# facebookresearch/r3m

Measured on AMD Instinct MI355X. Metric: encoder frames/sec (fwd+bwd) ResNet-50 224^2 bs=256/GPU, higher is better.
Workload: dtype f32

## Files before the change

### include/r3m_hip.h

```cpp
#ifndef R3M_HIP_H
#define R3M_HIP_H
#include <stddef.h>
#ifdef __cplusplus
extern "C" {
#endif

typedef void* r3m_stream_t;
typedef struct r3m_resnet* r3m_resnet_t;

int r3m_abi_version(void);
const char* r3m_last_error(void);

int r3m_debug_occupancy(int* out4);
int r3m_debug_occupy(int blocks, int lds_bytes, double milliseconds, r3m_stream_t stream);
int r3m_debug_set_dynamic_tiles(int on);
void r3m_debug_next_launch_tile_queues(unsigned* counters, int sets);
int r3m_debug_set_pw16(int mode);
int r3m_debug_set_conv3x3_bf16(int mode);
int r3m_debug_set_fused_inference(int on);
int r3m_debug_conv_route(int N, int H, int W, int Ci, int Co, int k, int stride, int pad, int dgrad, int flags, int mask_bits, int dtype,
                         int* routes, int cap);
int r3m_debug_conv_fuses_affine(int N, int H, int W, int Ci, int Co, int k, int stride, int pad, int flags, int dtype);
int r3m_debug_wgrad_route(int N, int H, int W, int Ci, int Co, int k, int stride, int pad, int dtype, int* out, int cap);
int r3m_debug_bn_geometry(long long rows, int C, int dtype, int* out, int cap);
void r3m_profile_enable(int on);
unsigned r3m_profile_classes(unsigned mask);
int r3m_profile_collect(double* ms, long long* launches, double* flops);
int r3m_profile_collect_bytes(double* bytes);
int r3m_profile_dump_to(const char* host_path);

r3m_resnet_t r3m_resnet_create(int size , int frames);
void r3m_resnet_destroy(r3m_resnet_t h);
int r3m_resnet_out_dim(r3m_resnet_t h);
long long r3m_resnet_num_params(r3m_resnet_t h);
long long r3m_resnet_num_buffers(r3m_resnet_t h);
long long r3m_resnet_arena_bytes(r3m_resnet_t h);
// ... 192 lines not shown
```

### r3m_amd/_lib.py

```python
import ctypes as C
import os

_HERE = os.path.dirname(os.path.abspath(__file__))
LIB_PATH = os.environ.get("R3M_HIP_LIB") or os.path.join(_HERE, "lib", "libr3m_hip.so")

_lib = None

c_f = C.c_void_p
c_i = C.c_int
c_ll = C.c_longlong
c_sz = C.c_size_t
c_fl = C.c_float
c_d = C.c_double

SIGNATURES = {
    "r3m_abi_version": (c_i, []),
    "r3m_last_error": (C.c_char_p, []),
    "r3m_debug_occupancy": (c_i, [C.POINTER(c_i)]),
    "r3m_debug_occupy": (c_i, [c_i, c_i, C.c_double, C.c_void_p]),
    "r3m_debug_set_dynamic_tiles": (c_i, [c_i]),
    "r3m_debug_next_launch_tile_queues": (None, [c_f, c_i]),
    "r3m_debug_set_pw16": (c_i, [c_i]),
    "r3m_debug_set_conv3x3_bf16": (c_i, [c_i]),
    "r3m_debug_set_fused_inference": (c_i, [c_i]),
    "r3m_debug_conv_route": (c_i, [c_i] * 12 + [C.POINTER(c_i), c_i]),
    "r3m_debug_wgrad_route": (c_i, [c_i] * 9 + [C.POINTER(c_i), c_i]),
    "r3m_debug_conv_fuses_affine": (c_i, [c_i] * 10),
    "r3m_debug_bn_geometry": (c_i, [c_ll, c_i, c_i, C.POINTER(c_i), c_i]),
    "r3m_profile_enable": (None, [c_i]),
    "r3m_profile_classes": (C.c_uint, [C.c_uint]),
    "r3m_profile_collect": (c_i, [C.POINTER(c_d), C.POINTER(c_ll), C.POINTER(c_d)]),
    "r3m_profile_collect_bytes": (c_i, [C.POINTER(c_d)]),
    "r3m_profile_dump_to": (c_i, [C.c_char_p]),
    "r3m_resnet_create": (C.c_void_p, [c_i, c_i]),
    "r3m_resnet_destroy": (None, [C.c_void_p]),
    "r3m_resnet_out_dim": (c_i, [C.c_void_p]),
    "r3m_resnet_num_params": (c_ll, [C.c_void_p]),
    "r3m_resnet_num_buffers": (c_ll, [C.c_void_p]),
    "r3m_resnet_arena_bytes": (c_ll, [C.c_void_p]),
    "r3m_resnet_num_tensors": (c_i, [C.c_void_p]),
# ... 189 lines not shown
```

### r3m_amd/csrc/capi.hip

```cpp
#include "engine.h"
#include "augment_dev.h"
#include "../../include/r3m_hip.h"
#include <cstdarg>
#include <cstdio>
#include <cstdlib>
#include <cstring>
#include <atomic>
#include <deque>
#include <mutex>
#include <string>
#include <vector>

namespace r3m {

static thread_local char g_err[512] = "";

void set_last_error(const char* fmt, ...) {
  va_list ap;
  va_start(ap, fmt);
  vsnprintf(g_err, sizeof g_err, fmt, ap);
  va_end(ap);
}

static int trace_mode() {
// ... 90 lines not shown
int r3m_debug_occupy(int blocks, int lds_bytes, double milliseconds, r3m_stream_t stream) {
  R3M_REQUIRE(blocks > 0 && lds_bytes >= 256 && lds_bytes <= 160 * 1024 && milliseconds >= 0.0, "debug_occupy: bad arguments");
  static r3m::DynLdsOptIn oi;
  if (int e = r3m::ensure_dyn_lds(oi, reinterpret_cast<const void*>(occupy_kernel), lds_bytes, "debug_occupy")) return e;
  hipLaunchKernelGGL(occupy_kernel, dim3(blocks), dim3(256), lds_bytes, static_cast<hipStream_t>(stream), (long long)(milliseconds * 1e5));
  return r3m::check_launch("debug_occupy");
}
int r3m_debug_set_dynamic_tiles(int on) { return r3m::gg_set_dynamic_tiles(on); }
void r3m_debug_next_launch_tile_queues(unsigned* counters, int sets) { r3m::gg_set_tile_counters(counters, counters && sets > 0 ? sets : 0); }
int r3m_debug_set_pw16(int mode) { return r3m::pw16_set_mode(mode); }
int r3m_debug_set_conv3x3_bf16(int mode) { return r3m::row16_set_mode(mode); }
int r3m_debug_set_fused_inference(int on) { return r3m::engine_set_fused_inference(on); }
int r3m_debug_conv_fuses_affine(int N, int H, int W, int Ci, int Co, int k, int stride, int pad, int flags, int dtype) {
  return r3m::conv_forward_affine_fusable({N, H, W, Ci, Co, k, stride, pad}, flags, dtype) ? 1 : 0;
}
int r3m_debug_conv_route(int N, int H, int W, int Ci, int Co, int k, int stride, int pad, int dgrad, int flags, int mask_bits, int dtype,
                         int* routes, int cap) {
  R3M_REQUIRE(routes && cap >= 1, "debug_conv_route: routes buffer");
  const unsigned* some_bits = reinterpret_cast<const unsigned*>(static_cast<uintptr_t>(64));
  const r3m::ConvGeom g{N, H, W, Ci, Co, k, stride, pad};
  r3m::gg_route_record_begin(routes, cap);
  int rc;
  if (!dgrad && (flags & EPI_AFFINE)) {
    const float* coef = reinterpret_cast<const float*>(some_bits);
    rc = r3m::conv_forward_launch_affine(nullptr, nullptr, nullptr, coef, coef, g, flags, dtype, nullptr);
  } else if (!dgrad) {
    rc = r3m::conv_forward_launch(nullptr, nullptr, nullptr, nullptr, nullptr, g, flags, dtype, nullptr);
  } else {
    r3m::BnRedArgs br{nullptr, mask_bits ? some_bits : nullptr, nullptr, nullptr, nullptr, nullptr, 0};
    const bool bn = (flags & 64) != 0;
    rc = r3m::conv_dgrad_launch(nullptr, nullptr, nullptr, nullptr, nullptr, (flags & 4) ? some_bits : nullptr, g, flags & ~64, dtype, nullptr,
                                bn ? &br : nullptr);
  }
  const int n = r3m::gg_route_record_end();
  return rc ? -1 : n;
}
int r3m_debug_wgrad_route(int N, int H, int W, int Ci, int Co, int k, int stride, int pad, int dtype, int* out, int cap) {
  if (!out || cap < 9) { r3m::set_last_error("debug_wgrad_route: the output buffer needs 9 ints"); return -1; }
  const r3m::WgradPlan r = r3m::conv_wgrad_plan({N, H, W, Ci, Co, k, stride, pad}, dtype);
  const int v[9] = {r.route, r.tile, r.bk, r.fast, r.split, r.rows_per_split, r.tilesN, r.gx, r.lds_bytes};
  for (int i = 0; i < 9; ++i) out[i] = v[i];
  return 9;
}
void r3m_profile_enable(int on) {
  std::lock_guard<std::mutex> lk(g_prof_mu);
  g_prof_on.store(on != 0, std::memory_order_relaxed);
  if (!on) g_prof_used = 0;
}
unsigned r3m_profile_classes(unsigned mask) { return g_prof_classes.exchange(mask, std::memory_order_relaxed); }
static FILE* g_prof_dump = nullptr;
// ... 554 lines not shown
```

### r3m_amd/csrc/common.h

```cpp
#pragma once
#include <hip/hip_runtime.h>
#include <stdint.h>
#include <stddef.h>

#ifdef R3M_PROBES
#include <cstdlib>
#define R3M_ENV_INT(name, dflt) ([]() -> int { static const int v_ = []() { const char* e_ = getenv(name); return e_ ? atoi(e_) : (dflt); }(); return v_; }())
#define R3M_PROBE(p) ((p).debug)
#else
#define R3M_ENV_INT(name, dflt) (dflt)
#define R3M_PROBE(p) 0
#endif

namespace r3m {

typedef float f32x4 __attribute__((ext_vector_type(4)));
typedef float f32x16 __attribute__((ext_vector_type(16)));

void set_last_error(const char* fmt, ...);
int  check_launch(const char* what);

#define R3M_REQUIRE(cond, ...)                  \
  do {                                          \
    if (!(cond)) {                              \
// ... 82 lines not shown
int launch_gather_gemm(const GatherGemmParams& p, hipStream_t s);
double gather_gemm_alg_bytes(const GatherGemmParams& p, int elem_bytes);
bool gather_gemm_fuses_affine(const GatherGemmParams& p);
int gather_gemm_grid_m(int M, int Nc);
void gg_set_tile_counters(unsigned* ctr8, int sets = 1);
int gg_set_dynamic_tiles(int on);
void gg_route_record_begin(int* out, int cap);
int gg_route_record_end();
struct WtEntry { long long w_off, wt_off; int Co, T, Ci, pad_; };
int launch_transpose_w_all(const float* params, void* wt, const WtEntry* tab, const int* tile0, int n, int tiles, int dt, hipStream_t s);
int launch_transpose_w(const float* W, float* Wt, int Co, int T, int Ci, hipStream_t s);

bool pw_gemm_eligible(const GatherGemmParams& p);
int pw_gemm_form(const GatherGemmParams& p);
int launch_pw_gemm(const GatherGemmParams& p, hipStream_t s);

enum : int {
  WG_TAPS_SIMPLE = 40,
  WG_TAPS_GATHER = 41,
  WG_ROWS        = 42,
  WG_WINDOW      = 43,
  WG16_TAPS      = 50,
  WG16_ROWS      = 51,
  WG16_ALL_TAPS  = 52,
};
struct WgradPlan {
  int route, tile, bk;
  int fast;
  int split, rows_per_split;
  int tilesN, gx;
// ... 151 lines not shown
```

### r3m_amd/csrc/conv.hip

```cpp
#include "common.h"
#include "conv_dev.h"
#include <utility>

namespace r3m {

__device__ __attribute__((aligned(128))) float g_zero_line[2048 + 64];


template <int EPI>
__global__ __launch_bounds__(256) void gather_gemm_glds_kernel(const GatherGemmParams p) {
  constexpr int BM = 128, BN = 128, WM = 2, WN = 2, TM = 2, TN = 2;
  constexpr int STAGE = (BM + BN) * 32;
  __shared__ __attribute__((aligned(128))) float smem[2 * STAGE];

  const int tid = threadIdx.x;
  const int lane = tid & 63;
  const int wave = tid >> 6;
  const int wm = wave / WN, wn = wave % WN;
  const int gridN = (p.Nc + BN - 1) / BN;
  const int lid = xcd_remap(blockIdx.x, gridDim.x);
  const int mt = lid / gridN, nt = lid % gridN;
  const int m0 = mt * BM, n0 = nt * BN;

  const int srow = lane >> 3;
// ... 749 lines not shown

  gg_epilogue<BM, BN, WM, WN, EPI, LDSB / 4>(p, acc, reinterpret_cast<float*>(wsm), m0, n0, mt);
}

static bool conv3x3_win_eligible(const GatherGemmParams& p, int maxW) {
  if (p.ntaps != 9 || p.is != 1 || p.os != 1 || p.simple_rows || p.Hg != p.Hi || p.Wg != p.Wi || p.Ho != p.Hi || p.Wo != p.Wi) return false;
  if (p.Wi > maxW || p.Wi < 1 || (p.Ci & 31)) return false;
  unsigned seen = 0;
  for (int t = 0; t < 9; ++t) {
    if (p.dy[t] < -1 || p.dy[t] > 1 || p.dx[t] < -1 || p.dx[t] > 1) return false;
    seen |= 1u << ((p.dy[t] + 1) * 3 + (p.dx[t] + 1));
  }
  return seen == 0x1ffu && (long long)p.Nc * p.T * p.Ci * 4 < 0x7FFFF000LL;
}

static inline bool gg_wide(int Nc) { return (Nc % 128) == 0; }

int gather_gemm_grid_m(int M, int Nc) { return gg_wide(Nc) ? ceil_div(M, 128) : ceil_div(M, 256); }

static int gg_use_glds() {
  const int v = R3M_ENV_INT("R3M_GG_GLDS", 2);
  return v;
}

#define GG_EPI_SWITCH(LAUNCH)                                                       \
  switch (p.flags) {                                                                \
    case 0: LAUNCH(0); break;                                                       \
    case EPI_STATS: LAUNCH(EPI_STATS); break;                                       \
    case EPI_ACCUM: LAUNCH(EPI_ACCUM); break;                                       \
    case EPI_MASKED_ADD: LAUNCH(EPI_MASKED_ADD); break;                             \
// ... 50 lines not shown
  p.debug = R3M_ENV_INT("R3M_GG_DEBUG", 0);
}

bool gather_gemm_fuses_affine(const GatherGemmParams& p_in) {
  GatherGemmParams p = p_in;
  gg_prepare(p);
  if (p.dtype == DT_BF16) return (p.Nc & 7) == 0 && (p.Ci & 63) == 0 && gg16_route_builds(gg16_route(p), p.flags);
  const int r = gg_route(p);
  if (r == GG_ROUTE_WIN) return p.flags == (EPI_AFFINE | EPI_RELU) || p.flags == (EPI_AFFINE | EPI_ACCUM | EPI_RELU);
  return r > GG_ROUTE_PW && r < GG_ROUTE_K16;
}
static thread_local int* t_route_out = nullptr;
static thread_local int t_route_n = 0, t_route_cap = 0;
void gg_route_record_begin(int* out, int cap) { t_route_out = out; t_route_n = 0; t_route_cap = cap; }
int gg_route_record_end() { const int n = t_route_n; t_route_out = nullptr; t_route_n = t_route_cap = 0; return n; }
static int gg_route_record(int route) {
  if (t_route_n < t_route_cap) t_route_out[t_route_n] = route;
  ++t_route_n;
  return 0;
}

enum : int { GG_OTHER_GLDS, GG_OTHER_NARROW, GG_OTHER_REG };
static int gg_other_kernel(bool wide) {
  if (!wide) return GG_OTHER_NARROW;
#ifdef R3M_PROBES
  if (!gg_use_glds()) return GG_OTHER_REG;
#endif
  return GG_OTHER_GLDS;
}

int launch_gather_gemm(const GatherGemmParams& p_in, hipStream_t s) {
  GatherGemmParams p = p_in;
  p.tile_ctr = t_tile_ctr;
  if (t_tile_ctr && --t_tile_ctr_sets > 0) t_tile_ctr += 8;
  else { t_tile_ctr = nullptr; t_tile_ctr_sets = 0; }
  R3M_REQUIRE(p.ntaps >= 0 && p.ntaps <= MAX_TAPS, "gather_gemm: ntaps=%d", p.ntaps);
  R3M_REQUIRE(p.M > 0 && p.Nc > 0, "gather_gemm: empty problem M=%d Nc=%d", p.M, p.Nc);
  gg_prepare(p);
  if (p.dtype == DT_BF16) {
    if (t_route_out) return gg_route_record(gg16_route(p));
    return launch_gather_gemm_bf16(p, s);
  }
  R3M_REQUIRE(p.Ci % 32 == 0, "gather_gemm: Ci=%d must be a multiple of 32", p.Ci);
  R3M_REQUIRE(p.Nc % 4 == 0, "gather_gemm: Nc=%d must be a multiple of 4", p.Nc);
  R3M_REQUIRE((reinterpret_cast<uintptr_t>(p.A) & 15) == 0 && (reinterpret_cast<uintptr_t>(p.B) & 15) == 0 &&
                  (reinterpret_cast<uintptr_t>(p.out) & 15) == 0,
              "gather_gemm: operands must be 16-byte aligned");
  const int route = gg_route(p);
  if (t_route_out) return gg_route_record(route);
  const bool wide = gg_wide(p.Nc);
  const int grid = wide ? ceil_div(p.M, 128) * ceil_div(p.Nc, 128) : ceil_div(p.M, 256) * ceil_div(p.Nc, 64);
  const double flops = 2.0 * (double)p.M * (double)p.Nc * ((double)p.ntaps * p.Ci);
  prof_begin(wide ? KC_GEMM_WIDE : KC_GEMM_NARROW, flops, p.M, p.Nc, p.Ci, p.ntaps, s);
  const char* what = "gather_gemm";
#define LAUNCH_GG(...) hipLaunchKernelGGL((__VA_ARGS__), dim3(grid), dim3(256), 0, s, p)
  switch (route) {
    case GG_ROUTE_WIN: {
      typedef WinCfg<128, 128, 192> Cfg;
#define LAUNCH_WIN(E)                                                                                                        \
  do {                                                                                                                       \
    static DynLdsOptIn oi;                                                                                                   \
    if (int e = ensure_dyn_lds(oi, reinterpret_cast<const void*>(conv3x3_win_kernel<128, 128, 2, 2, 192, E>), Cfg::LDS, "conv3x3_win")) return e; \
    hipLaunchKernelGGL((conv3x3_win_kernel<128, 128, 2, 2, 192, E>), dim3(grid), dim3(256), Cfg::LDS, s, p);                 \
  } while (0)
      switch (p.flags) {
        case EPI_AFFINE | EPI_RELU: LAUNCH_WIN(EPI_AFFINE | EPI_RELU); break;
        case EPI_AFFINE | EPI_ACCUM | EPI_RELU: LAUNCH_WIN(EPI_AFFINE | EPI_ACCUM | EPI_RELU); break;
        default:
          GG_EPI_SWITCH(LAUNCH_WIN)
      }
#undef LAUNCH_WIN
      what = "conv3x3_win";
// ... 117 lines not shown
```

### r3m_amd/csrc/conv_dev.h

```cpp
#pragma once
#include "common.h"
#include <utility>

namespace r3m {

typedef __bf16 bf16_t;
typedef __bf16 bf16x4 __attribute__((ext_vector_type(4)));
typedef __bf16 bf16x8 __attribute__((ext_vector_type(8)));

__device__ __forceinline__ f32x4 ld4t(const float* p) { return *reinterpret_cast<const f32x4*>(p); }
__device__ __forceinline__ f32x4 ld4t(const bf16_t* p) { return __builtin_convertvector(*reinterpret_cast<const bf16x4*>(p), f32x4); }
__device__ __forceinline__ void st4t(float* p, f32x4 v) { *reinterpret_cast<f32x4*>(p) = v; }
__device__ __forceinline__ void st4t(bf16_t* p, f32x4 v) { *reinterpret_cast<bf16x4*>(p) = __builtin_convertvector(v, bf16x4); }

__device__ __forceinline__ f32x4 ldg4(const float* p) { return *reinterpret_cast<const f32x4*>(p); }

#ifndef R3M_EPI_NT
#define R3M_EPI_NT 0
#endif
typedef unsigned int epi_u32x2 __attribute__((ext_vector_type(2)));
typedef unsigned int epi_u32x4 __attribute__((ext_vector_type(4)));
__device__ __forceinline__ void st4_out(float* p, f32x4 v) {
#if R3M_EPI_NT
  __builtin_nontemporal_store(v, reinterpret_cast<f32x4*>(p));
#else
  *reinterpret_cast<f32x4*>(p) = v;
#endif
}
__device__ __forceinline__ void st4_out(bf16_t* p, f32x4 v) {
#if R3M_EPI_NT
  __builtin_nontemporal_store(__builtin_bit_cast(epi_u32x2, __builtin_convertvector(v, bf16x4)), reinterpret_cast<epi_u32x2*>(p));
#else
  *reinterpret_cast<bf16x4*>(p) = __builtin_convertvector(v, bf16x4);
#endif
}
constexpr unsigned BUF_OOB = 0x7FFFF000u;
__device__ __forceinline__ void buf_store16(void* base, int bytes, unsigned voff, epi_u32x4 v) {
#if defined(__HIP_DEVICE_COMPILE__)
  __builtin_amdgcn_raw_buffer_store_b128(v, __builtin_amdgcn_make_buffer_rsrc(base, 0, bytes, 0x00020000), voff, 0, R3M_EPI_NT ? 2 : 0);
#endif
}
__device__ __forceinline__ epi_u32x4 buf_load16(const void* base, int bytes, unsigned voff) {
#if defined(__HIP_DEVICE_COMPILE__)
  return __builtin_amdgcn_raw_buffer_load_b128(__builtin_amdgcn_make_buffer_rsrc(const_cast<void*>(base), 0, bytes, 0x00020000), voff, 0, 0);
#else
  return epi_u32x4{0u, 0u, 0u, 0u};
#endif
}
__device__ __forceinline__ void st8_out(bf16_t* p, bf16x8 v) {
#if R3M_EPI_NT
  __builtin_nontemporal_store(__builtin_bit_cast(epi_u32x4, v), reinterpret_cast<epi_u32x4*>(p));
// ... 545 lines not shown
```

### r3m_amd/csrc/conv_pw.hip

```cpp
#include "common.h"
#include "conv_dev.h"

namespace r3m {

constexpr int PW_RSRC_FLAGS = 0x00020000;

__device__ __forceinline__ float pw_ld(const void* base, int bytes, unsigned voff, int soff) {
#if defined(__HIP_DEVICE_COMPILE__)
  return __builtin_bit_cast(float, __builtin_amdgcn_raw_buffer_load_b32(
                                       __builtin_amdgcn_make_buffer_rsrc(const_cast<void*>(base), 0, bytes, PW_RSRC_FLAGS), voff, soff, 0));
#else
  return 0.f;
#endif
}
__device__ __forceinline__ unsigned pw_ldu(const void* base, int bytes, unsigned voff, int soff) {
#if defined(__HIP_DEVICE_COMPILE__)
  return __builtin_amdgcn_raw_buffer_load_b32(__builtin_amdgcn_make_buffer_rsrc(const_cast<void*>(base), 0, bytes, PW_RSRC_FLAGS), voff, soff, 0);
#else
  return 0u;
#endif
}
typedef unsigned pw_u32x4 __attribute__((ext_vector_type(4)));
__device__ __forceinline__ f32x4 pw_ld4(const void* base, int bytes, unsigned voff, int soff) {
#if defined(__HIP_DEVICE_COMPILE__)
// ... 22 lines not shown
#endif
}
__device__ __forceinline__ void pw_st(void* base, int bytes, unsigned voff, int soff, float v) {
#if defined(__HIP_DEVICE_COMPILE__)
  __builtin_amdgcn_raw_buffer_store_b32(__builtin_bit_cast(unsigned, v), __builtin_amdgcn_make_buffer_rsrc(base, 0, bytes, PW_RSRC_FLAGS), voff,
                                        soff, 0);
#endif
}

__device__ __forceinline__ const float* pw_uniform_ptr(const float* q) {
  const unsigned long long v = reinterpret_cast<unsigned long long>(q);
  const unsigned lo = __builtin_amdgcn_readfirstlane((unsigned)v), hi = __builtin_amdgcn_readfirstlane((unsigned)(v >> 32));
  return reinterpret_cast<const float*>(((unsigned long long)hi << 32) | lo);
}

template <int BM, int BN, int WM, int WN, int EPI, bool YBITS = false, bool GATHER = false, bool OSTR = false, bool BURST = false>
__global__ __launch_bounds__(WM * WN * 64, WM * WN == 4 ? 2 : 1) void pw_gemm_kernel(const GatherGemmParams p, const int tiles, const int gridN) {
  constexpr int NW = WM * WN, TN = BN / WN / 32;
  static_assert(BM / WM == 64 && (TN == 1 || TN == 2) && (NW == 4 || NW == 8), "wave tile is 64 rows x 32 TN columns");
  constexpr int STAGE = (BM + BN) * 32;
  constexpr int AJ = BM / (8 * NW), BJ = BN / (8 * NW), NP = AJ + BJ;
  static_assert(AJ >= 1 && BJ >= 1 && (NP <= 8 || BURST), "a wave stages whole DMA instructions, at most one per odd MFMA slot (burst: any number)");
  constexpr int NST = 8 * TN;
  constexpr int SR = BN >= 128 ? 128 : 256, R = BM / SR;
  static_assert(R >= 1 && WM % R == 0 && (WM / R) * 64 == SR, "wave rows nest in statistics rows");
  extern __shared__ __attribute__((aligned(128))) float smem[];

  const int tid = threadIdx.x, lane = tid & 63;
  const int wave_s = __builtin_amdgcn_readfirstlane(tid >> 6);
  const int wm = wave_s / WN, wn = wave_s % WN;
  const int W = gridDim.x;
  const int K = p.Ci, Nc = p.Nc, Kb = K * 4;
  const int lrow = lane & 31, lh = lane >> 5;

  unsigned voffA[AJ], voffB[BJ];
  const int KbB = (GATHER ? p.T : 1) * Kb;
  {
    const int srow = lane >> 3, pslot = lane & 7;
#pragma unroll
    for (int j = 0; j < AJ; ++j) {
      const int r = wave_s * (BM / NW) + j * 8 + srow;
      voffA[j] = (unsigned)(r * Kb + ((pslot ^ ((r >> 1) & 7)) << 4));
    }
#pragma unroll
    for (int j = 0; j < BJ; ++j) {
      const int r = wave_s * (BN / NW) + j * 8 + srow;
      voffB[j] = (unsigned)(r * KbB + ((pslot ^ ((r >> 1) & 7)) << 4));
    }
// ... 8 lines not shown
      buf_dma16_uniform(dA, dAbytes, smem + STG * STAGE + wave_s * (BM / NW) * 32 + pc * 8 * 32, voffA[pc], dsA);
    else
      buf_dma16_uniform(dB, BN * KbB, smem + STG * STAGE + BM * 32 + wave_s * (BN / NW) * 32 + (pc - AJ) * 8 * 32, voffB[pc - AJ], dsB);
  };
  auto dma_all = [&](auto stg_c) __attribute__((always_inline)) {
    static_for<NP>([&](auto pc_c) __attribute__((always_inline)) { dma_piece(stg_c, pc_c); });
  };
  unsigned poff[GATHER ? AJ : 1], iyx[GATHER ? AJ : 1];
  int tap_soffB = 0;
  auto aim_tile = [&](int tmt_, int tnt_) __attribute__((always_inline)) {
    const int tmt = __builtin_amdgcn_readfirstlane(tmt_), tnt = __builtin_amdgcn_readfirstlane(tnt_);
    dB = p.B + (long long)tnt * BN * (KbB / 4);
    if constexpr (!GATHER) {
      dA = p.A + (long long)tmt * BM * K;
      dAbytes = min(BM, p.M - tmt * BM) * Kb;
    } else {
      const int hw = p.Hg * p.Wg;
      const int m0t = tmt * BM;
      const int nf = __builtin_amdgcn_readfirstlane(m0t / hw);
      const long long frame = (long long)p.Hi * p.Wi * K;
      dA = pw_uniform_ptr(p.A + nf * frame);
      const long long rest = (long long)(p.N - nf) * frame * 4;
      dAbytes = __builtin_amdgcn_readfirstlane(rest < (long long)BUF_OOB ? (int)rest : (int)BUF_OOB);
      const int srow = lane >> 3, pslot = lane & 7;
      const int r0 = wave_s * (BM / NW) + srow;
      int m = m0t + r0;
      int n = m / hw;
      int rem = m - n * hw;
      int gy = rem / p.Wg;
      int gx = rem - gy * p.Wg;
// ... 19 lines not shown
        }
      }
    }
  };
  auto set_tap = [&](int t) __attribute__((always_inline)) {
    if constexpr (GATHER) {
      const int pack = __builtin_amdgcn_readfirstlane(p.tap[t]);
      const int dy = (pack << 24) >> 24, dx = (pack << 16) >> 24, wt = pack >> 16;
      const int delta = (dy * p.Wi + dx) * Kb;
      tap_soffB = wt * Kb;
#pragma unroll
      for (int j = 0; j < AJ; ++j) {
        const unsigned iy = (iyx[j] >> 16) + (unsigned)dy, ix = (iyx[j] & 0xFFFFu) + (unsigned)dx;
        voffA[j] = (iy < (unsigned)p.Hi && ix < (unsigned)p.Wi) ? poff[j] + (unsigned)delta : BUF_OOB;
      }
    }
  };
  auto aim_step = [&](int chunk) __attribute__((always_inline)) {
    dsA = __builtin_amdgcn_readfirstlane(chunk * 128);
    dsB = __builtin_amdgcn_readfirstlane(tap_soffB + chunk * 128);
  };

  const float* fa[4];
  const float* fb[4];
  {
    const int xr = (lrow >> 1) & 7;
#pragma unroll
    for (int g = 0; g < 4; ++g) {
      const int go = ((2 * g + lh) ^ xr) * 4;
      fa[g] = smem + (wm * 64 + lrow) * 32 + go;
// ... 15 lines not shown
  f32x4 pg[PRE ? NST : 1], py[PRE ? NST : 1];
  typedef unsigned u32x2 __attribute__((ext_vector_type(2)));
  u32x2 pgm = {0u, 0u}, pym = {0u, 0u};
  const float* t_gb = nullptr;
  const float* t_yb = nullptr;
  const unsigned* t_gbits = nullptr;
  const unsigned* t_ybits = nullptr;
  int t_obytes = 0, t_bbytes = 0;
  static_assert(!OSTR || (GATHER && !MADD && !YBITS), "strided output rows: gather form, no mask words");
  unsigned orows[OSTR ? NST : 1];
  long long t_eo = 0;
  auto pre_tile = [&](int tmt, int tnt) __attribute__((always_inline)) {
    if constexpr (OSTR) {
      const int m0 = tmt * BM, n0 = tnt * BN;
      const int hw = p.Hg * p.Wg;
      const int nf = __builtin_amdgcn_readfirstlane(m0 / hw);
      const long long oframe = (long long)p.Ho * p.Wo * Nc;
      t_eo = nf * oframe + n0;
      const long long rest = ((long long)(p.N - nf) * oframe - n0) * 4;
      t_obytes = __builtin_amdgcn_readfirstlane(rest < (long long)BUF_OOB ? (int)rest : (int)BUF_OOB);
      const int m = m0 + wm * 64 + lane;
      const int n = m / hw;
      const int rem = m - n * hw;
      const int gy = rem / p.Wg, gx = rem - gy * p.Wg;
      const unsigned mine = m < p.M ? (unsigned)(((((n - nf) * p.Ho + gy * p.os + p.ooy) * p.Wo + gx * p.os + p.oox) * Nc) * 4) : BUF_OOB;
#pragma unroll
      for (int st = 0; st < NST; ++st)
        orows[st] = (unsigned)__builtin_amdgcn_ds_bpermute(4 * (st * RPS + srow), (int)mine) + (unsigned)((wn * TN * 32 + scol) * 4);
      if constexpr (ACC) t_gb = p.out + t_eo;
      if constexpr (BNR) t_yb = p.bn_y + t_eo;
    } else if constexpr (PRE) {
      const int m0 = tmt * BM, n0 = tnt * BN;
      const int rows_valid = min(BM, p.M - m0);
      const long long eo0 = (long long)m0 * Nc + n0;
      t_obytes = ((rows_valid - 1) * Nc + BN) * 4;
      t_bbytes = ((rows_valid - 1) * Nw + BN / 32) * 4;
      if constexpr (MADD) { t_gb = p.add0 + eo0; t_gbits = p.addbits + (eo0 >> 5); }
      if constexpr (ACC) t_gb = p.out + eo0;
      if constexpr (BNR) { t_yb = p.bn_y + eo0; t_ybits = YBITS ? p.bn_bits + (eo0 >> 5) : nullptr; }
    }
// ... 13 lines not shown
          if constexpr (TN == 2) pgm = pw_ld2(t_gbits, t_bbytes, vow);
          else pgm[0] = pw_ldu(t_gbits, t_bbytes, vow, 0);
        }
        if constexpr (BNR && YBITS) {
          if constexpr (TN == 2) pym = pw_ld2(t_ybits, t_bbytes, vow);
          else pym[0] = pw_ldu(t_ybits, t_bbytes, vow, 0);
        }
      }
    }
  };

  auto kstep = [&](auto stgm_c, auto first_c, auto dma_c, auto pf_c, bool do_dma, bool do_pf) __attribute__((always_inline)) {
    constexpr int STG_M = decltype(stgm_c)::value, PF = decltype(pf_c)::value;
    constexpr bool FIRST = decltype(first_c)::value, DMA = decltype(dma_c)::value;
    using SD = std::integral_constant<int, STG_M ^ 1>;
    constexpr int FB = ((MADD && BNR) || (GATHER && BNR && AJ > 4)) ? 1 : 2;
    f32x4 af[FB][2], bf[FB][TN];
    auto frag_load = [&](auto g_c) __attribute__((always_inline)) {
      constexpr int g = decltype(g_c)::value;
#pragma unroll
      for (int t = 0; t < 2; ++t) af[g % FB][t] = *reinterpret_cast<const f32x4*>(fa[g] + STG_M * STAGE + t * 32 * 32);
#pragma unroll
      for (int t = 0; t < TN; ++t) bf[g % FB][t] = *reinterpret_cast<const f32x4*>(fb[g] + STG_M * STAGE + t * 32 * 32);
    };
    if constexpr (FB == 2) frag_load(std::integral_constant<int, 0>{});
    static_for<4>([&](auto g_c) __attribute__((always_inline)) {
      constexpr int g = decltype(g_c)::value;
      if constexpr (FB == 1) frag_load(g_c);
      if constexpr (FB == 2 && g < 3) frag_load(std::integral_constant<int, g + 1>{});
      const f32x4(&a)[2] = af[g % FB];
      const f32x4(&b)[TN] = bf[g % FB];
// ... 172 lines not shown
          const float* q = src + ((r * (WM / R) + w) * WN) * (8 * CW);
          s += q[0];
          ss += q[CW];
        }
        const long long srow = (long long)emt * R + r;
        if (srow * SR < p.M) {
          const int col = ent * BN + c;
          p.stats[(srow * 2 + 0) * Nc + col] = s;
          p.stats[(srow * 2 + 1) * Nc + col] = ss;
        }
      }
    }
  };

  const int hp = K >> 6;
  const int npairs = (GATHER ? p.ntaps : 1) * hp;
  using I0 = std::integral_constant<int, 0>;
  using I1 = std::integral_constant<int, 1>;
  using T_ = std::true_type;
  using F_ = std::false_type;
  using P1 = std::integral_constant<int, 1>;
  using P2 = std::integral_constant<int, 2>;
  const bool dyn = p.tile_ctr != nullptr;
  const int xq = blockIdx.x & 7;
  unsigned* ctr = dyn ? p.tile_ctr + xq : nullptr;
  int* nxt = reinterpret_cast<int*>(slabs + 2 * CW);
  const int gridM = tiles / gridN;
  auto ticket_tile = [&](int k, int& tmt, int& tnt) -> bool {
    const int kp = k / gridN;
    tnt = k - kp * gridN;
    tmt = kp * 8 + xq;
// ... 7 lines not shown
    __syncthreads();
    has = ticket_tile(__builtin_amdgcn_readfirstlane(*nxt), mt, nt);
  } else {
    id = xcd_remap(blockIdx.x, W);
    mt = id / gridN;
    nt = id - mt * gridN;
    dm = W / gridN;
    dn = W - dm * gridN;
    has = id < tiles;
  }

  bool pending = false;
  int pmt = 0, pnt = 0;
  if (has) {
    aim_tile(mt, nt);
    set_tap(0);
    aim_step(0);
    dma_all(I0{});
  }
  while (true) {
    unsigned ticket = 0u;
    if (has) {
      asm volatile("s_waitcnt vmcnt(0)" ::: "memory");
      __syncthreads();
      aim_step(1);
      dma_all(I1{});
      if (dyn && tid == 0) ticket = __hip_atomic_fetch_add(ctr, 1u, __ATOMIC_RELAXED, __HIP_MEMORY_SCOPE_AGENT);
    }
    if (pending) epilogue1(pmt, pnt);
    if (!has) break;
    pre_tile(mt, nt);
    kstep(I0{}, T_{}, F_{}, P1{}, false, npairs == 1);
    int nid = id + W;
    int nmt = mt + dm, nnt = nt + dn;
    if (nnt >= gridN) { nnt -= gridN; ++nmt; }
    bool nhas = nid < tiles;
    int ti = 0, cp = 0;
    for (int pr = 0; pr < npairs; ++pr) {
      const bool last = pr + 1 == npairs;
      if (pr > 0) {
        asm volatile("s_waitcnt vmcnt(0)" ::: "memory");
        __syncthreads();
        aim_step(2 * cp + 1);
        if constexpr (BURST) {
          dma_all(I1{});
          kstep(I0{}, F_{}, F_{}, P1{}, false, last);
        } else if (R3M_PROBE(p) & 32) {
          dma_all(I1{});
          kstep(I0{}, F_{}, F_{}, P1{}, false, last);
        } else {
          kstep(I0{}, F_{}, T_{}, P1{}, true, last);
        }
      }
      if (pr == 0 && dyn && tid == 0) *nxt = (int)ticket;
      asm volatile("s_waitcnt vmcnt(0)" ::: "memory");
      __syncthreads();
      if (pr == 0 && dyn) nhas = ticket_tile(__builtin_amdgcn_readfirstlane(*nxt), nmt, nnt);
      if (pr == 0 && pending) epilogue2(pmt, pnt);
      bool do_dma = true;
      if (last) {
        do_dma = nhas;
        if (nhas) {
          aim_tile(nmt, nnt);
          set_tap(0);
          aim_step(0);
        }
      } else if (cp + 1 == hp) {
        set_tap(ti + 1);
        aim_step(0);
      } else {
        aim_step(2 * cp + 2);
      }
      if constexpr (BURST) {
        if (do_dma) dma_all(I0{});
        kstep(I1{}, F_{}, F_{}, P2{}, false, last);
      } else if (R3M_PROBE(p) & 32) {
        if (do_dma) dma_all(I0{});
        kstep(I1{}, F_{}, F_{}, P2{}, false, last);
      } else {
        kstep(I1{}, F_{}, T_{}, P2{}, do_dma, last);
      }
      if (++cp == hp) { cp = 0; ++ti; }
    }
// ... 55 lines not shown
    return 3;
  }
  if ((p.Nc & 127) == 0 && (p.flags & EPI_BNRED) && ((p.flags & EPI_MASKED_ADD) || p.bn_bits)) return 0;
  return 2;
}
bool pw_gemm_eligible(const GatherGemmParams& p) { return pw_gemm_form(p) != 0; }

static bool pw_burst(const GatherGemmParams& p) {
  const long long ktot = (long long)(p.simple_rows ? 1 : p.ntaps) * p.Ci;
  return (p.Nc & 127) != 0 && ktot >= 2LL * p.Nc &&
         (p.flags == EPI_STATS || p.flags == 0 || p.flags == (EPI_AFFINE | EPI_RELU) || (p.flags == EPI_BNRED && !p.bn_bits));
}

static bool pw_tile512() { return R3M_ENV_INT("R3M_PW_512", 1) != 0; }

template <int BM, int BN, int WM, int WN, bool GA, bool OS = false>
static int launch_pw_shape(const GatherGemmParams& p_in, hipStream_t s) {
  constexpr int NW = WM * WN, TN = BN / WN / 32;
  const int gridM = ceil_div(p_in.M, BM), gridN = p_in.Nc / BN;
  const long long tiles_ll = (long long)gridM * gridN;
  R3M_REQUIRE(tiles_ll < 0x7FFFFFFFLL, "pw_gemm: too many tiles");
  const int tiles = (int)tiles_ll;
  const int slots = (NW == 4 ? (BN == 64 ? 3 : 2) : 1) * pw_cu_count();
  const int W = tiles < slots ? tiles : slots;
  GatherGemmParams p = p_in;
  if (W < 64 || gridM < 64) p.tile_ctr = nullptr;
  constexpr int LDS = (2 * (BM + BN) * 32 + NW * 8 * TN * 32) * 4;
  static_assert(LDS <= 160 * 1024, "one CU's LDS");
  constexpr bool BURST_ONLY = BM / (8 * NW) + BN / (8 * NW) > 8;
#define LAUNCH_PW(E, YB)                                                                                                            \
  do {                                                                                                                             \
    static DynLdsOptIn oi;                                                                                                         \
    if (int e = ensure_dyn_lds(oi, reinterpret_cast<const void*>(pw_gemm_kernel<BM, BN, WM, WN, E, YB, GA, OS>), LDS, "pw_gemm")) return e; \
    hipLaunchKernelGGL((pw_gemm_kernel<BM, BN, WM, WN, E, YB, GA, OS>), dim3(W), dim3(NW * 64), LDS, s, p, tiles, gridN);               \
  } while (0)
#define LAUNCH_PW_BURST(E)                                                                                                          \
  do {                                                                                                                             \
    static DynLdsOptIn oi;                                                                                                         \
    if (int e = ensure_dyn_lds(oi, reinterpret_cast<const void*>(pw_gemm_kernel<BM, BN, WM, WN, E, false, GA, false, true>), LDS, "pw_gemm")) return e; \
    hipLaunchKernelGGL((pw_gemm_kernel<BM, BN, WM, WN, E, false, GA, false, true>), dim3(W), dim3(NW * 64), LDS, s, p, tiles, gridN);   \
  } while (0)
  const bool yb = p.bn_bits != nullptr;
  if constexpr (OS) {
    switch (p.flags) {
      case 0: LAUNCH_PW(0, false); return 0;
      case EPI_ACCUM: LAUNCH_PW(EPI_ACCUM, false); return 0;
      case EPI_BNRED: if (!yb) { LAUNCH_PW(EPI_BNRED, false); return 0; }
    }
    set_last_error("pw_gemm: form not built");
    return 1;
  } else {
  if constexpr (NW == 8) if (pw_burst(p)) {
    switch (p.flags) {
      case 0: LAUNCH_PW_BURST(0); return 0;
      case EPI_STATS: LAUNCH_PW_BURST(EPI_STATS); return 0;
      case EPI_AFFINE | EPI_RELU: LAUNCH_PW_BURST(EPI_AFFINE | EPI_RELU); return 0;
      case EPI_BNRED: LAUNCH_PW_BURST(EPI_BNRED); return 0;
    }
  }
  if constexpr (BURST_ONLY) {
    set_last_error("pw_gemm: form not built");
// ... 13 lines not shown
      else { set_last_error("pw_gemm: form not built"); return 1; }
      break;
    case EPI_BNRED | EPI_MASKED_ADD:
      if constexpr (!(GA && NW == 4)) {
        if (yb) LAUNCH_PW(EPI_BNRED | EPI_MASKED_ADD, true); else LAUNCH_PW(EPI_BNRED | EPI_MASKED_ADD, false);
      } else { set_last_error("pw_gemm: form not built"); return 1; }
      break;
    default: set_last_error("pw_gemm: unsupported epilogue flag combination %d", p.flags); return 1;
  }
  return 0;
  }
#undef LAUNCH_PW
#undef LAUNCH_PW_BURST
}

int launch_pw_gemm(const GatherGemmParams& p, hipStream_t s) {
  const bool wide = (p.Nc & 127) == 0;
  const int form = pw_gemm_form(p);
  if (form == 3) return wide ? launch_pw_shape<128, 128, 2, 2, true, true>(p, s) : launch_pw_shape<256, 64, 4, 2, true, true>(p, s);
  if (!wide && pw_burst(p) && pw_tile512()) return form == 2 ? launch_pw_shape<512, 64, 8, 1, true>(p, s) : launch_pw_shape<512, 64, 8, 1, false>(p, s);
  if (form == 2) return wide ? launch_pw_shape<128, 128, 2, 2, true>(p, s) : launch_pw_shape<256, 64, 4, 2, true>(p, s);
  return wide ? launch_pw_shape<128, 128, 2, 2, false>(p, s) : launch_pw_shape<256, 64, 4, 2, false>(p, s);
}

}
```

Before: 4238.

## Order 3x3 conv tiles per output pixel to skip padded taps

Adds a per-pixel tile ordering for small 3x3 stride-1 f32 convolutions (spatial size up to 14x14). Each 128-row tile covers the same output pixel across 128 frames, so the whole tile shares one valid-tap mask and taps that fall in padding are skipped. The route goes through the gather form of the pw_gemm kernel with per-row output offsets. It only engages when the skipped work outweighs the loss of spatial locality. In exchange it adds a strided output write pattern, more template instantiations and a single fragment buffer for the BN-reduce epilogue, plus a debug API that reports the pixel-order route.

```diff
diff --git a/include/r3m_hip.h b/include/r3m_hip.h
--- a/include/r3m_hip.h
+++ b/include/r3m_hip.h
@@ -20,6 +20,8 @@
 int r3m_debug_set_fused_inference(int on);
 int r3m_debug_conv_route(int N, int H, int W, int Ci, int Co, int k, int stride, int pad, int dgrad, int flags, int mask_bits, int dtype,
                          int* routes, int cap);
+int r3m_debug_conv_pixel_order(int N, int H, int W, int Ci, int Co, int k, int stride, int pad, int dgrad, int flags, int mask_bits, int dtype,
+                               int* masks, int cap);
 int r3m_debug_conv_fuses_affine(int N, int H, int W, int Ci, int Co, int k, int stride, int pad, int flags, int dtype);
 int r3m_debug_wgrad_route(int N, int H, int W, int Ci, int Co, int k, int stride, int pad, int dtype, int* out, int cap);
 int r3m_debug_bn_geometry(long long rows, int C, int dtype, int* out, int cap);
diff --git a/r3m_amd/_lib.py b/r3m_amd/_lib.py
--- a/r3m_amd/_lib.py
+++ b/r3m_amd/_lib.py
@@ -24,6 +24,7 @@
     "r3m_debug_set_conv3x3_bf16": (c_i, [c_i]),
     "r3m_debug_set_fused_inference": (c_i, [c_i]),
     "r3m_debug_conv_route": (c_i, [c_i] * 12 + [C.POINTER(c_i), c_i]),
+    "r3m_debug_conv_pixel_order": (c_i, [c_i] * 12 + [C.POINTER(c_i), c_i]),
     "r3m_debug_wgrad_route": (c_i, [c_i] * 9 + [C.POINTER(c_i), c_i]),
     "r3m_debug_conv_fuses_affine": (c_i, [c_i] * 10),
     "r3m_debug_bn_geometry": (c_i, [c_ll, c_i, c_i, C.POINTER(c_i), c_i]),
diff --git a/r3m_amd/csrc/capi.hip b/r3m_amd/csrc/capi.hip
--- a/r3m_amd/csrc/capi.hip
+++ b/r3m_amd/csrc/capi.hip
@@ -128,9 +128,8 @@
 int r3m_debug_conv_fuses_affine(int N, int H, int W, int Ci, int Co, int k, int stride, int pad, int flags, int dtype) {
   return r3m::conv_forward_affine_fusable({N, H, W, Ci, Co, k, stride, pad}, flags, dtype) ? 1 : 0;
 }
-int r3m_debug_conv_route(int N, int H, int W, int Ci, int Co, int k, int stride, int pad, int dgrad, int flags, int mask_bits, int dtype,
-                         int* routes, int cap) {
-  R3M_REQUIRE(routes && cap >= 1, "debug_conv_route: routes buffer");
+static int conv_route_dry_run(int N, int H, int W, int Ci, int Co, int k, int stride, int pad, int dgrad, int flags, int mask_bits, int dtype,
+                              int* routes, int cap) {
   const unsigned* some_bits = reinterpret_cast<const unsigned*>(static_cast<uintptr_t>(64));
   const r3m::ConvGeom g{N, H, W, Ci, Co, k, stride, pad};
   r3m::gg_route_record_begin(routes, cap);
@@ -146,8 +145,22 @@
     rc = r3m::conv_dgrad_launch(nullptr, nullptr, nullptr, nullptr, nullptr, (flags & 4) ? some_bits : nullptr, g, flags & ~64, dtype, nullptr,
                                 bn ? &br : nullptr);
   }
+  return rc;
+}
+int r3m_debug_conv_route(int N, int H, int W, int Ci, int Co, int k, int stride, int pad, int dgrad, int flags, int mask_bits, int dtype,
+                         int* routes, int cap) {
+  R3M_REQUIRE(routes && cap >= 1, "debug_conv_route: routes buffer");
+  const int rc = conv_route_dry_run(N, H, W, Ci, Co, k, stride, pad, dgrad, flags, mask_bits, dtype, routes, cap);
   const int n = r3m::gg_route_record_end();
   return rc ? -1 : n;
+}
+int r3m_debug_conv_pixel_order(int N, int H, int W, int Ci, int Co, int k, int stride, int pad, int dgrad, int flags, int mask_bits, int dtype,
+                               int* masks, int cap) {
+  int routes[4];
+  const int rc = conv_route_dry_run(N, H, W, Ci, Co, k, stride, pad, dgrad, flags, mask_bits, dtype, routes, 4);
+  const int taken = rc ? -1 : r3m::gg_pixel_order_last(masks, masks ? cap : 0);
+  const int n = r3m::gg_route_record_end();
+  return rc ? -1 : (n == 1 ? taken : 0);
 }
 int r3m_debug_wgrad_route(int N, int H, int W, int Ci, int Co, int k, int stride, int pad, int dtype, int* out, int cap) {
   if (!out || cap < 9) { r3m::set_last_error("debug_wgrad_route: the output buffer needs 9 ints"); return -1; }
diff --git a/r3m_amd/csrc/common.h b/r3m_amd/csrc/common.h
--- a/r3m_amd/csrc/common.h
+++ b/r3m_amd/csrc/common.h
@@ -120,6 +120,9 @@
 bool pw_gemm_eligible(const GatherGemmParams& p);
 int pw_gemm_form(const GatherGemmParams& p);
 int launch_pw_gemm(const GatherGemmParams& p, hipStream_t s);
+bool pw_pixel_fits(const GatherGemmParams& p);
+int launch_pw_pixel(const GatherGemmParams& p, hipStream_t s);
+int gg_pixel_order_last(int* masks, int cap);
 
 enum : int {
   WG_TAPS_SIMPLE = 40,
diff --git a/r3m_amd/csrc/conv.hip b/r3m_amd/csrc/conv.hip
--- a/r3m_amd/csrc/conv.hip
+++ b/r3m_amd/csrc/conv.hip
@@ -787,6 +787,17 @@
   return seen == 0x1ffu && (long long)p.Nc * p.T * p.Ci * 4 < 0x7FFFF000LL;
 }
 
+constexpr int PIX_MAX_HW = 14 * 14;
+static bool conv3x3_pixel_eligible(const GatherGemmParams& p) {
+  if (!R3M_ENV_INT("R3M_GG_PIX", 1)) return false;
+  if (!conv3x3_win_eligible(p, 28) || !pw_pixel_fits(p)) return false;
+  const long long hw = (long long)p.Hi * p.Wi;
+  if (hw > R3M_ENV_INT("R3M_GG_PIX_HW", PIX_MAX_HW)) return false;
+  const long long valid = (3LL * p.Hi - 2) * (3LL * p.Wi - 2);
+  const long long whole = p.N / 128;
+  return whole * 128 * valid + (p.N - whole * 128) * hw * 9 < (long long)p.N * hw * 9;
+}
+
 static inline bool gg_wide(int Nc) { return (Nc % 128) == 0; }
 
 int gather_gemm_grid_m(int M, int Nc) { return gg_wide(Nc) ? ceil_div(M, 128) : ceil_div(M, 256); }
@@ -867,10 +878,21 @@
 static thread_local int t_route_n = 0, t_route_cap = 0;
 void gg_route_record_begin(int* out, int cap) { t_route_out = out; t_route_n = 0; t_route_cap = cap; }
 int gg_route_record_end() { const int n = t_route_n; t_route_out = nullptr; t_route_n = t_route_cap = 0; return n; }
-static int gg_route_record(int route) {
+static thread_local GatherGemmParams t_route_last;
+static thread_local int t_route_last_route = 0;
+static int gg_route_record(int route, const GatherGemmParams& p) {
   if (t_route_n < t_route_cap) t_route_out[t_route_n] = route;
   ++t_route_n;
+  t_route_last = p;
+  t_route_last_route = route;
   return 0;
+}
+int gg_pixel_order_last(int* masks, int cap) {
+  const GatherGemmParams& p = t_route_last;
+  if (!t_route_out || t_route_n < 1 || p.dtype != DT_F32 || t_route_last_route != GG_ROUTE_WIN) return 0;
+  const int np = p.Ho * p.Wo < cap ? p.Ho * p.Wo : cap;
+  for (int i = 0; masks && i < np; ++i) masks[i] = (int)pixel_tap_mask(p.tap, p.ntaps, i / p.Wo, i % p.Wo, p.Hi, p.Wi);
+  return conv3x3_pixel_eligible(p) ? 1 : 0;
 }
 
 enum : int { GG_OTHER_GLDS, GG_OTHER_NARROW, GG_OTHER_REG };
@@ -891,7 +913,7 @@
   R3M_REQUIRE(p.M > 0 && p.Nc > 0, "gather_gemm: empty problem M=%d Nc=%d", p.M, p.Nc);
   gg_prepare(p);
   if (p.dtype == DT_BF16) {
-    if (t_route_out) return gg_route_record(gg16_route(p));
+    if (t_route_out) return gg_route_record(gg16_route(p), p);
     return launch_gather_gemm_bf16(p, s);
   }
   R3M_REQUIRE(p.Ci % 32 == 0, "gather_gemm: Ci=%d must be a multiple of 32", p.Ci);
@@ -900,7 +922,7 @@
                   (reinterpret_cast<uintptr_t>(p.out) & 15) == 0,
               "gather_gemm: operands must be 16-byte aligned");
   const int route = gg_route(p);
-  if (t_route_out) return gg_route_record(route);
+  if (t_route_out) return gg_route_record(route, p);
   const bool wide = gg_wide(p.Nc);
   const int grid = wide ? ceil_div(p.M, 128) * ceil_div(p.Nc, 128) : ceil_div(p.M, 256) * ceil_div(p.Nc, 64);
   const double flops = 2.0 * (double)p.M * (double)p.Nc * ((double)p.ntaps * p.Ci);
@@ -909,6 +931,11 @@
 #define LAUNCH_GG(...) hipLaunchKernelGGL((__VA_ARGS__), dim3(grid), dim3(256), 0, s, p)
   switch (route) {
     case GG_ROUTE_WIN: {
+      if (conv3x3_pixel_eligible(p)) {
+        if (int e = launch_pw_pixel(p, s)) return e;
+        what = "pw_gemm";
+        break;
+      }
       typedef WinCfg<128, 128, 192> Cfg;
 #define LAUNCH_WIN(E)                                                                                                        \
   do {                                                                                                                       \
diff --git a/r3m_amd/csrc/conv_dev.h b/r3m_amd/csrc/conv_dev.h
--- a/r3m_amd/csrc/conv_dev.h
+++ b/r3m_amd/csrc/conv_dev.h
@@ -35,6 +35,15 @@
 #endif
 }
 constexpr unsigned BUF_OOB = 0x7FFFF000u;
+__host__ __device__ inline unsigned pixel_tap_mask(const int* tap, int ntaps, int py, int px, int Hi, int Wi) {
+  unsigned m = 0u;
+  for (int t = 0; t < ntaps; ++t) {
+    const int pack = tap[t];
+    const int dy = (pack << 24) >> 24, dx = (pack << 16) >> 24;
+    if ((unsigned)(py + dy) < (unsigned)Hi && (unsigned)(px + dx) < (unsigned)Wi) m |= 1u << t;
+  }
+  return m;
+}
 __device__ __forceinline__ void buf_store16(void* base, int bytes, unsigned voff, epi_u32x4 v) {
 #if defined(__HIP_DEVICE_COMPILE__)
   __builtin_amdgcn_raw_buffer_store_b128(v, __builtin_amdgcn_make_buffer_rsrc(base, 0, bytes, 0x00020000), voff, 0, R3M_EPI_NT ? 2 : 0);
diff --git a/r3m_amd/csrc/conv_pw.hip b/r3m_amd/csrc/conv_pw.hip
--- a/r3m_amd/csrc/conv_pw.hip
+++ b/r3m_amd/csrc/conv_pw.hip
@@ -60,7 +60,8 @@
   return reinterpret_cast<const float*>(((unsigned long long)hi << 32) | lo);
 }
 
-template <int BM, int BN, int WM, int WN, int EPI, bool YBITS = false, bool GATHER = false, bool OSTR = false, bool BURST = false>
+template <int BM, int BN, int WM, int WN, int EPI, bool YBITS = false, bool GATHER = false, bool OSTR = false, bool BURST = false,
+          bool PIX = false>
 __global__ __launch_bounds__(WM * WN * 64, WM * WN == 4 ? 2 : 1) void pw_gemm_kernel(const GatherGemmParams p, const int tiles, const int gridN) {
   constexpr int NW = WM * WN, TN = BN / WN / 32;
   static_assert(BM / WM == 64 && (TN == 1 || TN == 2) && (NW == 4 || NW == 8), "wave tile is 64 rows x 32 TN columns");
@@ -78,6 +79,10 @@
   const int W = gridDim.x;
   const int K = p.Ci, Nc = p.Nc, Kb = K * 4;
   const int lrow = lane & 31, lh = lane >> 5;
+  static_assert(!PIX || (GATHER && OSTR && BM == 128 && NW == 4), "per-pixel tile order: gather form, per-row result offsets, 128-row tile");
+  const int npix = PIX ? (p.N / BM) * (p.Hg * p.Wg) : 0;
+  unsigned smask = 0u;
+  int np_next = 0;
 
   unsigned voffA[AJ], voffB[BJ];
   const int KbB = (GATHER ? p.T : 1) * Kb;
@@ -116,6 +121,57 @@
     if constexpr (!GATHER) {
       dA = p.A + (long long)tmt * BM * K;
       dAbytes = min(BM, p.M - tmt * BM) * Kb;
+    } else if constexpr (PIX) {
+      const int hw = p.Hg * p.Wg;
+      const bool pxt = tmt < npix;
+      const int q = __builtin_amdgcn_readfirstlane((pxt ? tmt : tmt * BM) / hw);
+      const int pix = tmt - q * hw;
+      const int py = __builtin_amdgcn_readfirstlane(pix / p.Wg), px = pix - py * p.Wg;
+      const int nf = pxt ? q * BM : q;
+      const long long frame = (long long)p.Hi * p.Wi * K;
+      dA = pw_uniform_ptr(p.A + nf * frame);
+      const long long rest = (long long)(p.N - nf) * frame * 4;
+      dAbytes = __builtin_amdgcn_readfirstlane(rest < (long long)BUF_OOB ? (int)rest : (int)BUF_OOB);
+      const int srow = lane >> 3, pslot = lane & 7;
+      const int r0 = wave_s * (BM / NW) + srow;
+      if (pxt) {
+#pragma unroll
+        for (int j = 0; j < AJ; ++j) {
+          const int r = r0 + j * 8;
+          poff[j] = (unsigned)((((r * p.Hi + py) * p.Wi + px) * K) * 4 + ((pslot ^ ((r >> 1) & 7)) << 4));
+          iyx[j] = (unsigned)((py << 16) | px);
+        }
+      } else {
+        int m = tmt * BM + r0;
+        int n = m / hw;
+        int rem = m - n * hw;
+        int gy = rem / p.Wg;
+        int gx = rem - gy * p.Wg;
+#pragma unroll
+        for (int j = 0; j < AJ; ++j) {
+          const int r = r0 + j * 8;
+          poff[j] = (unsigned)(((((n - nf) * p.Hi + gy) * p.Wi + gx) * K) * 4 + ((pslot ^ ((r >> 1) & 7)) << 4));
+          iyx[j] = m < p.M ? (unsigned)((gy << 16) | gx) : 0x40004000u;
+          m += 8;
+          gx += 8;
+#pragma unroll
+          for (int w = 0; w < 2; ++w) {
+            const bool c = gx >= p.Wg;
+            gx -= c ? p.Wg : 0;
+            gy += c ? 1 : 0;
+          }
+#pragma unroll
+          for (int w = 0; w < 2; ++w) {
+            const bool c = gy >= p.Hg;
+            gy -= c ? p.Hg : 0;
+            n += c ? 1 : 0;
+          }
+        }
+      }
+      unsigned vm = (1u << p.ntaps) - 1u;
+      if (pxt && !(R3M_PROBE(p) & 64)) vm = pixel_tap_mask(p.tap, p.ntaps, py, px, p.Hi, p.Wi);
+      smask = __builtin_amdgcn_readfirstlane(vm);
+      np_next = __builtin_popcount(smask) * (K >> 6);
     } else {
       const int hw = p.Hg * p.Wg;
       const int m0t = tmt * BM;
@@ -165,6 +221,16 @@
         const unsigned iy = (iyx[j] >> 16) + (unsigned)dy, ix = (iyx[j] & 0xFFFFu) + (unsigned)dx;
         voffA[j] = (iy < (unsigned)p.Hi && ix < (unsigned)p.Wi) ? poff[j] + (unsigned)delta : BUF_OOB;
       }
+    }
+  };
+  int ti = 0;
+  auto tap_next = [&](bool first) __attribute__((always_inline)) -> int {
+    if constexpr (PIX) {
+      const int t = __builtin_ctz(smask);
+      smask &= smask - 1u;
+      return t;
+    } else {
+      return first ? 0 : ti + 1;
     }
   };
   auto aim_step = [&](int chunk) __attribute__((always_inline)) {
@@ -210,16 +276,22 @@
     if constexpr (OSTR) {
       const int m0 = tmt * BM, n0 = tnt * BN;
       const int hw = p.Hg * p.Wg;
-      const int nf = __builtin_amdgcn_readfirstlane(m0 / hw);
+      const int nf = __builtin_amdgcn_readfirstlane(PIX && m0 / BM < npix ? (m0 / BM) / hw * BM : m0 / hw);
       const long long oframe = (long long)p.Ho * p.Wo * Nc;
       t_eo = nf * oframe + n0;
       const long long rest = ((long long)(p.N - nf) * oframe - n0) * 4;
       t_obytes = __builtin_amdgcn_readfirstlane(rest < (long long)BUF_OOB ? (int)rest : (int)BUF_OOB);
       const int m = m0 + wm * 64 + lane;
-      const int n = m / hw;
-      const int rem = m - n * hw;
-      const int gy = rem / p.Wg, gx = rem - gy * p.Wg;
-      const unsigned mine = m < p.M ? (unsigned)(((((n - nf) * p.Ho + gy * p.os + p.ooy) * p.Wo + gx * p.os + p.oox) * Nc) * 4) : BUF_OOB;
+      unsigned mine;
+      if constexpr (PIX) {
+        const int pix = m0 / BM - (nf / BM) * hw;
+        mine = m0 / BM < npix ? (unsigned)(((wm * 64 + lane) * hw + pix) * Nc * 4) : m < p.M ? (unsigned)((m - nf * hw) * Nc * 4) : BUF_OOB;
+      } else {
+        const int n = m / hw;
+        const int rem = m - n * hw;
+        const int gy = rem / p.Wg, gx = rem - gy * p.Wg;
+        mine = m < p.M ? (unsigned)(((((n - nf) * p.Ho + gy * p.os + p.ooy) * p.Wo + gx * p.os + p.oox) * Nc) * 4) : BUF_OOB;
+      }
 #pragma unroll
       for (int st = 0; st < NST; ++st)
         orows[st] = (unsigned)__builtin_amdgcn_ds_bpermute(4 * (st * RPS + srow), (int)mine) + (unsigned)((wn * TN * 32 + scol) * 4);
@@ -263,7 +335,7 @@
     constexpr int STG_M = decltype(stgm_c)::value, PF = decltype(pf_c)::value;
     constexpr bool FIRST = decltype(first_c)::value, DMA = decltype(dma_c)::value;
     using SD = std::integral_constant<int, STG_M ^ 1>;
-    constexpr int FB = ((MADD && BNR) || (GATHER && BNR && AJ > 4)) ? 1 : 2;
+    constexpr int FB = ((MADD && BNR) || (GATHER && BNR && AJ > 4) || (PIX && BNR)) ? 1 : 2;
     f32x4 af[FB][2], bf[FB][TN];
     auto frag_load = [&](auto g_c) __attribute__((always_inline)) {
       constexpr int g = decltype(g_c)::value;
@@ -466,7 +538,7 @@
   };
 
   const int hp = K >> 6;
-  const int npairs = (GATHER ? p.ntaps : 1) * hp;
+  int npairs = (GATHER ? p.ntaps : 1) * hp;
   using I0 = std::integral_constant<int, 0>;
   using I1 = std::integral_constant<int, 1>;
   using T_ = std::true_type;
@@ -504,7 +576,7 @@
   int pmt = 0, pnt = 0;
   if (has) {
     aim_tile(mt, nt);
-    set_tap(0);
+    set_tap(tap_next(true));
     aim_step(0);
     dma_all(I0{});
   }
@@ -519,13 +591,15 @@
     }
     if (pending) epilogue1(pmt, pnt);
     if (!has) break;
+    if constexpr (PIX) npairs = np_next;
     pre_tile(mt, nt);
     kstep(I0{}, T_{}, F_{}, P1{}, false, npairs == 1);
     int nid = id + W;
     int nmt = mt + dm, nnt = nt + dn;
     if (nnt >= gridN) { nnt -= gridN; ++nmt; }
     bool nhas = nid < tiles;
-    int ti = 0, cp = 0;
+    int cp = 0;
+    ti = 0;
     for (int pr = 0; pr < npairs; ++pr) {
       const bool last = pr + 1 == npairs;
       if (pr > 0) {
@@ -552,11 +626,11 @@
         do_dma = nhas;
         if (nhas) {
           aim_tile(nmt, nnt);
-          set_tap(0);
+          set_tap(tap_next(true));
           aim_step(0);
         }
       } else if (cp + 1 == hp) {
-        set_tap(ti + 1);
+        set_tap(tap_next(false));
         aim_step(0);
       } else {
         aim_step(2 * cp + 2);
@@ -642,7 +716,7 @@
 
 static bool pw_tile512() { return R3M_ENV_INT("R3M_PW_512", 1) != 0; }
 
-template <int BM, int BN, int WM, int WN, bool GA, bool OS = false>
+template <int BM, int BN, int WM, int WN, bool GA, bool OS = false, bool PX = false>
 static int launch_pw_shape(const GatherGemmParams& p_in, hipStream_t s) {
   constexpr int NW = WM * WN, TN = BN / WN / 32;
   const int gridM = ceil_div(p_in.M, BM), gridN = p_in.Nc / BN;
@@ -659,8 +733,8 @@
 #define LAUNCH_PW(E, YB)                                                                                                            \
   do {                                                                                                                             \
     static DynLdsOptIn oi;                                                                                                         \
-    if (int e = ensure_dyn_lds(oi, reinterpret_cast<const void*>(pw_gemm_kernel<BM, BN, WM, WN, E, YB, GA, OS>), LDS, "pw_gemm")) return e; \
-    hipLaunchKernelGGL((pw_gemm_kernel<BM, BN, WM, WN, E, YB, GA, OS>), dim3(W), dim3(NW * 64), LDS, s, p, tiles, gridN);               \
+    if (int e = ensure_dyn_lds(oi, reinterpret_cast<const void*>(pw_gemm_kernel<BM, BN, WM, WN, E, YB, GA, OS, false, PX>), LDS, "pw_gemm")) return e; \
+    hipLaunchKernelGGL((pw_gemm_kernel<BM, BN, WM, WN, E, YB, GA, OS, false, PX>), dim3(W), dim3(NW * 64), LDS, s, p, tiles, gridN);               \
   } while (0)
 #define LAUNCH_PW_BURST(E)                                                                                                          \
   do {                                                                                                                             \
@@ -670,9 +744,10 @@
   } while (0)
   const bool yb = p.bn_bits != nullptr;
   if constexpr (OS) {
+    if constexpr (PX) if (p.flags == EPI_STATS) { LAUNCH_PW(EPI_STATS, false); return 0; }
     switch (p.flags) {
       case 0: LAUNCH_PW(0, false); return 0;
-      case EPI_ACCUM: LAUNCH_PW(EPI_ACCUM, false); return 0;
+      case EPI_ACCUM: if constexpr (!PX) { LAUNCH_PW(EPI_ACCUM, false); return 0; } else break;
       case EPI_BNRED: if (!yb) { LAUNCH_PW(EPI_BNRED, false); return 0; }
     }
     set_last_error("pw_gemm: form not built");
@@ -716,6 +791,19 @@
 #undef LAUNCH_PW_BURST
 }
 
+bool pw_pixel_fits(const GatherGemmParams& p) {
+  if (p.dtype != DT_F32 || (p.Ci & 63) || p.Ci > 2048 || (p.Nc & 127) || p.ntaps < 1 || p.ntaps > 9 || p.simple_rows) return false;
+  if (p.flags != EPI_STATS && p.flags != 0 && !(p.flags == EPI_BNRED && !p.bn_bits)) return false;
+  if (p.is != 1 || p.os != 1 || p.ooy != 0 || p.oox != 0 || p.Hg != p.Ho || p.Wg != p.Wo || p.Hg != p.Hi || p.Wg != p.Wi) return false;
+  if (p.Hi < 2 || p.Wi < 4 || p.Hi >= 16384 || p.Wi >= 16384) return false;
+  const long long frame = (long long)p.Hi * p.Wi * (p.Ci > p.Nc ? p.Ci : p.Nc) * 4;
+  return 130LL * frame < (long long)BUF_OOB && 128LL * p.T * p.Ci * 4 < (long long)BUF_OOB;
+}
+int launch_pw_pixel(const GatherGemmParams& p, hipStream_t s) {
+  R3M_REQUIRE(pw_pixel_fits(p), "pw_gemm: per-pixel tile order asked for a launch it does not take");
+  return launch_pw_shape<128, 128, 2, 2, true, true, true>(p, s);
+}
+
 int launch_pw_gemm(const GatherGemmParams& p, hipStream_t s) {
   const bool wide = (p.Nc & 127) == 0;
   const int form = pw_gemm_form(p);
```

After: 4267 (median of 6 runs). About the same (+0.7%).
